# kepingbi/ProdSearch

Hardware: AMD Instinct MI355X
Metric: train (u,q,i,neg) tuples/sec at bs=384, 20 neg, d=128 (higher is better)
Workload: dtype f32 (fp32 MFMA and VALU; wide products, the fused per-replica kernels and grouped weight gradients as fp32-grade bf16x3 products: exact 3-way bf16 split of both fp32 operands, 6 of the 9 cross products as bf16 MFMAs per step, fp32 accumulation); 1 GPU; item_transformer d=128 1 layer 8 heads ff=512 uprev=20 bs=384/GPU 20 neg Q=8 W=1 P=18357 V=32387 dropout=0.10 (BASELINE configs[1]); global_batch=384, parallelism=dp1, step=sample+fwd+bwd+clip/Adam via nn.Module API (trainer.py:74-78), replicas_per_row=21

## Files before the change

### include/prodsearch_hip.h

```cpp
#ifndef PRODSEARCH_HIP_H
#define PRODSEARCH_HIP_H

#include <stddef.h>
#include <stdint.h>

#ifdef __cplusplus
extern "C" {
#endif

#define PS_MAX_LAYERS 8
#define PS_OK 0
#define PS_ERR_ARG 1
#define PS_ERR_HIP 2

typedef void* ps_stream_t;

enum { PS_MODEL_TEM = 0, PS_MODEL_QEM = 1,
       PS_MODEL_AEM = 2,
       PS_MODEL_ZAM = 3 };
enum { PS_QENC_FS = 0, PS_QENC_AVG = 1 };

typedef struct PsTemDesc {
  int32_t B;
  int32_t K;
// ... 40 lines not shown
  float *fs_w, *fs_b;
  float *pe;
  float *final_ln_g, *final_ln_b;
  PsLayerTensors layer[PS_MAX_LAYERS];
} PsTemTensors;

typedef struct PsTemBatch {
  const int64_t *query_word_idxs;
  const int64_t *target_prod_idxs;
  const int64_t *u_item_idxs;
  const int64_t *pos_iword_idxs;
  const int64_t *neg_item_idxs;
  const int64_t *neg_word_idxs;
  const int64_t *candi_prod_idxs;
} PsTemBatch;

typedef struct PsTemWsLayout {
  int64_t total_floats;
  int32_t R;
  int32_t S;
  int64_t qmean, query_emb, x;
  int64_t kp, vp, qp, attn, ctx;
  int64_t y1, ln1, a1, h1, y2, enc;
  int64_t item_scores, word_scores, loss_parts;
  int64_t denc, dx;
} PsTemWsLayout;

const char* ps_version(void);
const char* ps_last_error(void);
const char* ps_arith_info(void);
int ps_set_fuse_bwd_min(int rows);
int ps_set_item_scatter_fused(int on);
int ps_item_scatter_fused_taken(void);
int ps_set_side_mode(int mode);
int ps_side_values_in_use(void);
void ps_side_abort(void);
void ps_debug_fail_fork(int nth);
int ps_set_deterministic(int on);
int ps_gemm_x3_config(int mode, int force_shape);
int ps_gemm_f32_weight(const float* A, int lda, const float* W, int tb, float* C, int ldc, int M, int N, int K,
                       const float* bias, float alpha, ps_stream_t stream);

int ps_tem_workspace_layout(const PsTemDesc* desc, PsTemWsLayout* out);

int ps_tem_forward(const PsTemDesc* desc, const PsTemTensors* params, const PsTemBatch* batch,
                   float* workspace, float* loss3, float* loss_acc, ps_stream_t stream);
int ps_tem_forward_sampled(const PsTemDesc* desc, const PsTemTensors* params, const PsTemBatch* batch,
                           const float* alias_prob, const int32_t* alias_idx, int64_t* neg_item_out, int64_t* neg_word_out,
                           float* workspace, float* loss3, float* loss_acc, ps_stream_t stream);

int ps_tem_backward(const PsTemDesc* desc, const PsTemTensors* params, const PsTemBatch* batch,
                    float* workspace, const PsTemTensors* grads, float loss_scale,
                    const float* loss_scale_dev ,
                    ps_stream_t stream);

int ps_gather_score(const PsTemDesc* desc, const PsTemTensors* params, const PsTemBatch* batch,
                    float* workspace, ps_stream_t stream);

int ps_tem_score(const PsTemDesc* desc, const PsTemTensors* params, const PsTemBatch* batch,
                 float* workspace, float* scores, ps_stream_t stream);

int ps_sample_negatives(const PsTemDesc* desc, const float* alias_prob, const int32_t* alias_idx,
                        int64_t* neg_item_idxs, int64_t* neg_word_idxs, ps_stream_t stream);
int ps_build_alias_host(const double* dist_host, int64_t n, float* prob_host, int32_t* alias_host);

typedef struct PsAdamHyper {
// ... 199 lines not shown
```

### prodsearch_amd/_lib.py

```python
import ctypes as C
import os

from . import build as _build

PS_MAX_LAYERS = 8
PS_MODEL_TEM, PS_MODEL_QEM, PS_MODEL_AEM, PS_MODEL_ZAM = 0, 1, 2, 3
PS_QENC_FS, PS_QENC_AVG = 0, 1

_f32p = C.POINTER(C.c_float)
_i64p = C.POINTER(C.c_int64)


class PsTemDesc(C.Structure):
    _fields_ = [(n, C.c_int32) for n in ('B', 'K', 'L', 'Q', 'W', 'C', 'd', 'H', 'F', 'n_layers')] + \
               [('product_size', C.c_int64), ('vocab_size', C.c_int64)] + \
               [(n, C.c_int32) for n in ('model', 'query_encoder', 'use_pos_emb', 'use_item_pos',
                                         'bias_product', 'pos_weight', 'sep_prod_emb', 'training')] + \
               [('dropout', C.c_float), ('seed', C.c_uint64), ('step', C.c_uint64)]


LAYER_FIELDS = ('wk', 'bk', 'wv', 'bv', 'wq', 'bq', 'wo', 'bo', 'w1', 'b1', 'w2', 'b2',
                'ff_ln_g', 'ff_ln_b', 'ln_g', 'ln_b')
TOP_FIELDS = ('product_emb', 'hist_product_emb', 'word_emb', 'product_bias', 'word_bias',
              'fs_w', 'fs_b', 'pe', 'final_ln_g', 'final_ln_b')
# ... 49 lines not shown

RTM_TOP_FIELDS = ('word_emb', 'review_emb', 'seg_emb', 'fs_w', 'fs_b', 'pe', 'final_ln_g', 'final_ln_b',
                  'wo_w', 'wo_b', 'user_emb', 'product_emb', 'rev_fs_w', 'rev_fs_b')
RTM_BATCH_FIELDS = ('query_word_idxs', 'pos_prod_ridxs', 'pos_seg_idxs', 'pos_prod_rword_idxs',
                    'pos_prod_rword_masks', 'neg_prod_ridxs', 'neg_seg_idxs', 'neg_prod_rword_idxs',
                    'pos_prod_rword_idxs_pvc', 'neg_prod_rword_idxs_pvc', 'neg_word_idxs',
                    'candi_prod_ridxs', 'candi_seg_idxs', 'review_embeddings', 'pos_user_idxs', 'neg_user_idxs',
                    'pos_item_idxs', 'neg_item_idxs', 'candi_seq_user_idxs', 'candi_seq_item_idxs', 'neg_prod_rword_masks')


class PsRtmTensors(C.Structure):
    _fields_ = [(n, C.c_void_p) for n in RTM_TOP_FIELDS] + [('layer', PsLayerTensors * PS_MAX_LAYERS)]


class PsRtmBatch(C.Structure):
    _fields_ = [(n, C.c_void_p) for n in RTM_BATCH_FIELDS]


class PsRtmWsLayout(C.Structure):
    _fields_ = [('total_floats', C.c_int64)] + [(n, C.c_int32) for n in ('Bseq', 'S', 'J', 'pad_')] + \
               [(n, C.c_int64) for n in ('query_emb', 'valid', 'x', 'vec', 'cnt', 'enc', 'scores', 'weight',
                                         'pv_scores', 'dx')]


PS_RENC_PV, PS_RENC_PVC, PS_RENC_FS, PS_RENC_AVG = 0, 1, 2, 3

SYMBOLS = {
    'ps_version': (C.c_char_p, []),
    'ps_last_error': (C.c_char_p, []),
    'ps_arith_info': (C.c_char_p, []),
    'ps_set_fuse_bwd_min': (C.c_int, [C.c_int]),
    'ps_set_item_scatter_fused': (C.c_int, [C.c_int]),
    'ps_item_scatter_fused_taken': (C.c_int, []),
    'ps_set_side_mode': (C.c_int, [C.c_int]),
    'ps_side_values_in_use': (C.c_int, []),
    'ps_set_deterministic': (C.c_int, [C.c_int]),
    'ps_side_abort': (None, []),
    'ps_debug_fail_fork': (None, [C.c_int]),
    'ps_gemm_x3_config': (C.c_int, [C.c_int, C.c_int]),
    'ps_gemm_f32_weight': (C.c_int, [C.c_void_p, C.c_int, C.c_void_p, C.c_int, C.c_void_p, C.c_int, C.c_int, C.c_int, C.c_int,
                                     C.c_void_p, C.c_float, C.c_void_p]),
    'ps_tem_workspace_layout': (C.c_int, [C.POINTER(PsTemDesc), C.POINTER(PsTemWsLayout)]),
    'ps_tem_forward': (C.c_int, [C.POINTER(PsTemDesc), C.POINTER(PsTemTensors), C.POINTER(PsTemBatch),
                                 C.c_void_p, C.c_void_p, C.c_void_p, C.c_void_p]),
    'ps_tem_forward_sampled': (C.c_int, [C.POINTER(PsTemDesc), C.POINTER(PsTemTensors), C.POINTER(PsTemBatch),
                                         C.c_void_p, C.c_void_p, C.c_void_p, C.c_void_p, C.c_void_p, C.c_void_p, C.c_void_p,
                                         C.c_void_p]),
    'ps_tem_backward': (C.c_int, [C.POINTER(PsTemDesc), C.POINTER(PsTemTensors), C.POINTER(PsTemBatch),
                                  C.c_void_p, C.POINTER(PsTemTensors), C.c_float, C.c_void_p, C.c_void_p]),
    'ps_gather_score': (C.c_int, [C.POINTER(PsTemDesc), C.POINTER(PsTemTensors), C.POINTER(PsTemBatch),
                                  C.c_void_p, C.c_void_p]),
    'ps_tem_score': (C.c_int, [C.POINTER(PsTemDesc), C.POINTER(PsTemTensors), C.POINTER(PsTemBatch),
                               C.c_void_p, C.c_void_p, C.c_void_p]),
    'ps_rtm_workspace_floats': (C.c_int, [C.POINTER(PsRtmDesc), C.c_int32, C.POINTER(C.c_int64)]),
    'ps_rtm_workspace_layout': (C.c_int, [C.POINTER(PsRtmDesc), C.c_int32, C.POINTER(PsRtmWsLayout)]),
    'ps_rtm_forward': (C.c_int, [C.POINTER(PsRtmDesc), C.POINTER(PsRtmTensors), C.POINTER(PsRtmBatch),
                                 C.c_void_p, C.c_void_p, C.c_void_p]),
    'ps_rtm_backward': (C.c_int, [C.POINTER(PsRtmDesc), C.POINTER(PsRtmTensors), C.POINTER(PsRtmBatch),
                                  C.c_void_p, C.POINTER(PsRtmTensors), C.c_float, C.c_void_p, C.c_void_p]),
    'ps_rtm_score': (C.c_int, [C.POINTER(PsRtmDesc), C.POINTER(PsRtmTensors), C.POINTER(PsRtmBatch),
                               C.c_void_p, C.c_void_p, C.c_void_p]),
    'ps_rtm_review_embeddings': (C.c_int, [C.POINTER(PsRtmDesc), C.POINTER(PsRtmTensors), C.c_void_p,
                                           C.c_void_p, C.c_void_p, C.c_void_p]),
    'ps_sample_negatives': (C.c_int, [C.POINTER(PsTemDesc), C.c_void_p, C.c_void_p, C.c_void_p,
                                      C.c_void_p, C.c_void_p]),
    'ps_build_alias_host': (C.c_int, [C.c_void_p, C.c_int64, C.c_void_p, C.c_void_p]),
# ... 171 lines not shown
```

### prodsearch_amd/csrc/mlp_fused.hip

```cpp
#include "rowwise.h"
#include "x3frag.h"
#include <stdlib.h>
#ifndef TRY
#define TRY(x) do { int _rc = (x); if (_rc) return _rc; } while (0)
#endif

bool ps_fusion_enabled() {
  static const bool on = ps_env_int("PS_NO_FUSE", 0) == 0;
  return on;
}

#define MD 128
#define MBM 32
#define MT_THREADS 512
#define MLP_PF_DEFAULT 3
#define PLD 132

__device__ inline int opaque(int v) { asm volatile("" : "+v"(v)); return v; }

struct MlpTLds {
  uint16_t Xa[3][MBM * MD];
  float Ps[8][MBM * PLD];
  float vec[6][MD];
  float red[16];
// ... 356 lines not shown
template <class K>
static int set_lds_attr(K kernel, bool& done) {
  if (!done) {
    PS_CHECK_HIP(hipFuncSetAttribute(reinterpret_cast<const void*>(kernel), hipFuncAttributeMaxDynamicSharedMemorySize, (int)sizeof(MlpTLds)));
    done = true;
  }
  return PS_OK;
}

int launch_mlp_fwd_fused(const MlpFwdArgs& a, hipStream_t st) {
  PS_REQUIRE(mlp_x3_enabled(a.F) && a.M > 0, "fused mlp: F=%d M=%d (F must be 256, 512 or 1024)", a.F, a.M);
  PS_REQUIRE(a.x3.on && a.x3.fwd_wo && a.x3.fwd_ff, "fused mlp: the weight fragment streams are missing (WSplit)");
  PS_REQUIRE(!a.fold_score || mlp_fwd_can_fold_score(a.M, a.F, MD), "fused mlp: folded scoring needs <= 65535 workgroups");
  KTimeScope kt("mlp_fwd", st);
  MlpFwdArgs as = a;
  as.stamp = g_mlp_stamp;
  const dim3 grid(ps_cdiv(a.M, MBM)), block(MT_THREADS);
  static bool a1 = false, a2 = false, a4 = false;
#ifdef PS_DIAG
  static bool ad1 = false, ad2 = false, ad3 = false;
  static const int diag = ps_diag_int("PS_MLP_DIAG", 0);
  if (a.F == 512 && diag == 1) { TRY(set_lds_attr(mlp_fwd_t_kernel<2, 3, 1>, ad1)); PS_KLAUNCH((mlp_fwd_t_kernel<2, 3, 1>), grid, block, sizeof(MlpTLds), st, as); }
  else if (a.F == 512 && diag == 2) { TRY(set_lds_attr(mlp_fwd_t_kernel<2, 3, 2>, ad2)); PS_KLAUNCH((mlp_fwd_t_kernel<2, 3, 2>), grid, block, sizeof(MlpTLds), st, as); }
  else if (a.F == 512 && diag == 3) { TRY(set_lds_attr(mlp_fwd_t_kernel<2, 3, 3>, ad3)); PS_KLAUNCH((mlp_fwd_t_kernel<2, 3, 3>), grid, block, sizeof(MlpTLds), st, as); }
  else
#endif
  if (a.F == 256) { TRY(set_lds_attr(mlp_fwd_t_kernel<1, 3>, a1)); PS_KLAUNCH((mlp_fwd_t_kernel<1, 3>), grid, block, sizeof(MlpTLds), st, as); }
  else if (a.F == 512) { TRY(set_lds_attr(mlp_fwd_t_kernel<2, 3>, a2)); PS_KLAUNCH((mlp_fwd_t_kernel<2, 3>), grid, block, sizeof(MlpTLds), st, as); }
  else { TRY(set_lds_attr(mlp_fwd_t_kernel<4, 3>, a4)); PS_KLAUNCH((mlp_fwd_t_kernel<4, 3>), grid, block, sizeof(MlpTLds), st, as); }
  PS_LAUNCH_CHECK();
  return PS_OK;
}

template <int NBW, int PF, bool ISC>
__global__ __launch_bounds__(MT_THREADS, 2) void mlp_bwd_t_kernel(const MlpBwdArgs a) {
  fork_signal(a.sig, a.sigval);
  extern __shared__ float lds_raw[];
  MlpTLds& L = *reinterpret_cast<MlpTLds*>(lds_raw);
  const int tid = threadIdx.x, lane = tid & 63, wave = __builtin_amdgcn_readfirstlane(tid >> 6), l31 = lane & 31, h = lane >> 5;
  const int m0 = blockIdx.x * MBM, M = a.M, F = a.F;
  const int mrow = 4 * wave + (lane >> 4), c8 = 8 * (lane & 15);
  const int mg = m0 + mrow;
  const bool ok = mg < M;
  const uint32_t step_ctx = drop_step(a.drop_ctx), step_ff1 = drop_step(a.drop_ff1), step_ff2 = drop_step(a.drop_ff2);
  MLP_STAMP(0);
  float (*Csum)[MBM][MD] = reinterpret_cast<float (*)[MBM][MD]>(&L.Ps[2][0]);
  static_assert(3 * MBM * MD <= 3 * MBM * PLD, "column-sum scratch must fit three partial slots");

  const uint16_t* ff_stream = a.x3.bwd_ff + (size_t)(wave * NBW) * 16 * 1536;
  uint4 ring[PF][3];
#pragma unroll
  for (int s = 0; s < PF; ++s) load_frag(ring[s], ff_stream, s, lane);
  if (tid < 64) {
    const int which = tid >> 5, q = tid & 31;
    *reinterpret_cast<float4*>(&L.vec[which][4 * q]) = *reinterpret_cast<const float4*>((which == 0 ? a.gf : a.g1) + 4 * q);
  }
  float isc_e[4][2], isc_ds[4]; int isc_idx[4]; bool isc_live[4];
  if (ISC) {
#pragma unroll
    for (int r = 0; r < 4; ++r) {
      const int mr = m0 + 4 * wave + r;
      const float* er = a.enc + (size_t)(mr < M ? mr : 0) * MD + lane;
      isc_e[r][0] = er[0]; isc_e[r][1] = er[64];
    }
  }
  auto isc_add = [&](const int r) {
    float* g = a.g_product_emb + (size_t)isc_idx[r] * MD + lane;
    atomicAdd(g, isc_live[r] ? isc_ds[r] * isc_e[r][0] : 0.f);
    atomicAdd(g + 64, isc_live[r] ? isc_ds[r] * isc_e[r][1] : 0.f);
    if (a.g_product_bias && lane == 0) atomicAdd(&a.g_product_bias[isc_idx[r]], isc_ds[r]);
  };
  float x2[8], st2[2] = {0.f, 0.f};
  {
    const float* src = a.y2 + (size_t)(ok ? mg : 0) * MD + c8;
    const float4 v0 = ok ? *reinterpret_cast<const float4*>(src) : make_float4(0.f, 0.f, 0.f, 0.f);
    const float4 v1 = ok ? *reinterpret_cast<const float4*>(src + 4) : make_float4(0.f, 0.f, 0.f, 0.f);
    x2[0] = v0.x; x2[1] = v0.y; x2[2] = v0.z; x2[3] = v0.w; x2[4] = v1.x; x2[5] = v1.y; x2[6] = v1.z; x2[7] = v1.w;
    if (ok) { const float2 s2 = *reinterpret_cast<const float2*>(a.stf + 2 * (size_t)mg); st2[0] = s2.x; st2[1] = s2.y; }
  }
  float dy[8];
  if (a.item_scores) {
    const float invB = a.scale * (a.scale_dev ? *a.scale_dev : 1.f) / (float)a.B;
    const float wpos = a.pos_weight ? (float)a.K : 1.f;
    const int K1 = a.K + 1;
    const int mm = ok ? mg : 0;
    const int b = mm / K1, j = mm - b * K1;
    int64_t idx = j == 0 ? a.target[b] : a.neg_items[(size_t)b * a.K + j - 1];
    idx = idx < 0 ? a.P : (idx > a.P ? a.P : idx);
    const float sc = a.item_scores[mm];
    const float ds = ok ? (j == 0 ? wpos * (sigmoid_f(sc) - 1.f) : sigmoid_f(sc)) * invB : 0.f;
    const float* row = a.product_emb + (size_t)idx * MD + c8;
    const float4 v0 = *reinterpret_cast<const float4*>(row), v1 = *reinterpret_cast<const float4*>(row + 4);
    dy[0] = ds * v0.x; dy[1] = ds * v0.y; dy[2] = ds * v0.z; dy[3] = ds * v0.w;
    dy[4] = ds * v1.x; dy[5] = ds * v1.y; dy[6] = ds * v1.z; dy[7] = ds * v1.w;
    if (ISC) {
#pragma unroll
      for (int r = 0; r < 4; ++r) {
        isc_ds[r] = __builtin_bit_cast(float, __builtin_amdgcn_readlane(__builtin_bit_cast(int, ds), 16 * r));
        isc_idx[r] = __builtin_amdgcn_readlane((int)idx, 16 * r);
        isc_live[r] = m0 + 4 * wave + r < M && isc_idx[r] != (int)a.P;
      }
    }
  } else {
    const float* src = a.denc + (size_t)(ok ? mg : 0) * MD + c8;
    const float4 v0 = ok ? *reinterpret_cast<const float4*>(src) : make_float4(0.f, 0.f, 0.f, 0.f);
    const float4 v1 = ok ? *reinterpret_cast<const float4*>(src + 4) : make_float4(0.f, 0.f, 0.f, 0.f);
    dy[0] = v0.x; dy[1] = v0.y; dy[2] = v0.z; dy[3] = v0.w; dy[4] = v1.x; dy[5] = v1.y; dy[6] = v1.z; dy[7] = v1.w;
  }
  __syncthreads();
  MLP_STAMP(1);

  auto ln_bwd_stage = [&](const float (&dyv)[8], const float (&x)[8], const float mean, const float rstd, const int vg,
                          const bool has_res, const float (&res)[8], const DropSpec& drop, const uint32_t dstep,
                          float (&dxr)[8], float* out_dx, float* out_drop) {
    const float4 g0 = *reinterpret_cast<const float4*>(&L.vec[vg][c8]), g1 = *reinterpret_cast<const float4*>(&L.vec[vg][c8 + 4]);
    const float gg[8] = {g0.x, g0.y, g0.z, g0.w, g1.x, g1.y, g1.z, g1.w};
    float xh[8], dh[8], s1 = 0.f, s2 = 0.f;
#pragma unroll
    for (int j = 0; j < 8; ++j) {
      xh[j] = (x[j] - mean) * rstd;
      dh[j] = dyv[j] * gg[j];
      s1 += dh[j]; s2 += dh[j] * xh[j];
    }
    s1 = row16_sum(s1) * (1.f / MD);
    s2 = row16_sum(s2) * (1.f / MD);
    Philox4 rnd = {0u, 0u, 0u, 0u};
    if (drop.thr) rnd = drop_call16(drop, (uint32_t)mg, (uint32_t)(lane & 15), dstep);
    float v[8];
#pragma unroll
    for (int j = 0; j < 8; ++j) {
      float dlt = rstd * (dh[j] - s1 - xh[j] * s2);
      if (has_res) dlt += res[j];
      if (!ok) dlt = 0.f;
      dxr[j] = dlt;
// ... 39 lines not shown
#pragma unroll
    for (int j = 0; j < 8; ++j) dyz[j] = ok ? dy[j] : 0.f;
    ln_bwd_stage(dyz, x2, st2[0], st2[1], 0, false, zero, a.drop_ff2, step_ff2, dy2r, nullptr, a.do2);
  }
  __syncthreads();
  MLP_STAMP(2);
  park(a.part_f);
  __syncthreads();
  MLP_STAMP(3);

  f32x16 acc2[4];
#pragma unroll
  for (int nb = 0; nb < 4; ++nb)
#pragma unroll
    for (int r = 0; r < 16; ++r) acc2[nb][r] = 0.f;
  const int mrow_p = m0 + l31;
  const bool row_ok = mrow_p < M;
  constexpr int NS = 16 * NBW;
#pragma unroll
  for (int bi = 0; bi < NBW; ++bi) {
    const int fb = wave * NBW + bi, f0 = 32 * fb + 16 * h;
    float* tile = &L.Ps[wave][0];
    float4 a1g[4];
    tile_load(a1g, a.a1 + (size_t)m0 * F + 32 * fb, F, lane, M - m0);
    f32x16 acc1;
#pragma unroll
    for (int r = 0; r < 16; ++r) acc1[r] = 0.f;
    uint4 bq[2][3];
    read_b(bq[0], L.Xa, l31, 8 * h);
    if (ISC) {
#pragma unroll
      for (int r = 0; r < 4; ++r) if (r * NBW / 2 == 2 * bi) isc_add(r);
    }
    { if ((wave >= 4) == (bi == 0)) __builtin_amdgcn_s_setprio(2); else __builtin_amdgcn_s_setprio(1); }
#pragma unroll
    for (int t = 0; t < 8; ++t) {
      const int s = 16 * bi + t;
      if (t + 1 < 8) read_b(bq[(t + 1) & 1], L.Xa, l31, 16 * (t + 1) + 8 * h);
      __builtin_amdgcn_sched_barrier(0);
      x3_mma(acc1, ring[s % PF], bq[t & 1]);
      load_frag(ring[s % PF], ff_stream, s + PF < NS ? s + PF : NS - 1, lane);
      __builtin_amdgcn_sched_barrier(0);
    }
    { if ((wave >= 4) == (bi == 0)) __builtin_amdgcn_s_setprio(1); else __builtin_amdgcn_s_setprio(0); }
    MLP_STAMP(4 + 2 * bi);
    Philox4 r0 = {0u, 0u, 0u, 0u}, r1 = {0u, 0u, 0u, 0u};
    if (a.drop_ff1.thr) {
      r0 = drop_call16(a.drop_ff1, (uint32_t)mrow_p, (uint32_t)(f0 >> 3), step_ff1);
      r1 = drop_call16(a.drop_ff1, (uint32_t)mrow_p, (uint32_t)(f0 >> 3) + 1u, step_ff1);
    }
    float a1v[16];
    tile_load_put(tile, a1g, lane);
    tile_get(tile, a1v, l31, h);
    float dv[16];
#pragma unroll
    for (int r = 0; r < 16; ++r) {
      float g = acc1[r] * gelu_tanh_grad(a1v[r]);
      if (a.drop_ff1.thr) g *= drop_half(a.drop_ff1, r < 8 ? r0 : r1, r & 7);
      dv[r] = row_ok ? g : 0.f;
    }
    tile_put(tile + MBM * TLD, dv, l31, h);
    tile_store(tile + MBM * TLD, a.da1 + (size_t)m0 * F + 32 * fb, F, lane, M - m0);
    {
      float cs[16];
#pragma unroll
      for (int r = 0; r < 16; ++r) cs[r] = half_sum_last(dv[r]);
      if (l31 == 31) {
        float* pb = a.part_b1 + ((size_t)blockIdx.x * 3) * F + f0;
#pragma unroll
        for (int q = 0; q < 4; ++q) *reinterpret_cast<float4*>(pb + 4 * q) = make_float4(cs[4 * q], cs[4 * q + 1], cs[4 * q + 2], cs[4 * q + 3]);
      }
    }
    MLP_STAMP(5 + 2 * bi);
    { if ((wave >= 4) == (bi == 0)) __builtin_amdgcn_s_setprio(2); else __builtin_amdgcn_s_setprio(1); }
    uint4 df[2][3];
    {
      const float lo8[8] = {dv[0], dv[1], dv[2], dv[3], dv[4], dv[5], dv[6], dv[7]};
      const float hi8[8] = {dv[8], dv[9], dv[10], dv[11], dv[12], dv[13], dv[14], dv[15]};
      split8(lo8, df[0]);
      split8(hi8, df[1]);
    }
    if (ISC) {
#pragma unroll
      for (int r = 0; r < 4; ++r) if (r * NBW / 2 == 2 * bi + 1) isc_add(r);
    }
#pragma unroll
    for (int u = 0; u < 8; ++u) {
      const int s = 16 * bi + 8 + u;
      x3_mma(acc2[u & 3], ring[s % PF], df[u >> 2]);
      load_frag(ring[s % PF], ff_stream, s + PF < NS ? s + PF : NS - 1, lane);
      __builtin_amdgcn_sched_barrier(0);
    }
  }
  __builtin_amdgcn_s_setprio(0);
  MLP_STAMP(8);
  float x1[8], st1v[2] = {0.f, 0.f};
  {
    const float* src = a.y1 + (size_t)(ok ? mg : 0) * MD + c8;
    const float4 v0 = ok ? *reinterpret_cast<const float4*>(src) : make_float4(0.f, 0.f, 0.f, 0.f);
    const float4 v1 = ok ? *reinterpret_cast<const float4*>(src + 4) : make_float4(0.f, 0.f, 0.f, 0.f);
    x1[0] = v0.x; x1[1] = v0.y; x1[2] = v0.z; x1[3] = v0.w; x1[4] = v1.x; x1[5] = v1.y; x1[6] = v1.z; x1[7] = v1.w;
    if (ok) { const float2 s2 = *reinterpret_cast<const float2*>(a.st1 + 2 * (size_t)mg); st1v[0] = s2.x; st1v[1] = s2.y; }
  }
  const int kbo = wave & 3, nh = wave >> 2;
  const uint16_t* wo_stream = a.x3.bwd_wo + (size_t)(kbo * 8 + 4 * nh) * 1536;
  uint4 wof[4][3];
#pragma unroll
  for (int t = 0; t < 4; ++t) load_frag(wof[t], wo_stream, t, lane);
#pragma unroll
  for (int nb = 0; nb < 4; ++nb) dump_acc(L.Ps[wave], acc2[nb], l31, h, nb);
  __syncthreads();
  MLP_STAMP(9);

  float dl[8] = {0.f, 0.f, 0.f, 0.f, 0.f, 0.f, 0.f, 0.f};
  for (int s = 0; s < 8; ++s) {
    const float* p = &L.Ps[s][mrow * PLD + c8];
    const float4 p0 = *reinterpret_cast<const float4*>(p), p1 = *reinterpret_cast<const float4*>(p + 4);
    dl[0] += p0.x; dl[1] += p0.y; dl[2] += p0.z; dl[3] += p0.w; dl[4] += p1.x; dl[5] += p1.y; dl[6] += p1.z; dl[7] += p1.w;
  }
  __syncthreads();
  MLP_STAMP(10);
  {
    float dy1r[8];
    const bool same = a.dout == a.dy1;
// ... 1 lines not shown
  }
  __syncthreads();
  MLP_STAMP(11);
  park(a.part_1);
  {
    f32x16 acc;
#pragma unroll
    for (int r = 0; r < 16; ++r) acc[r] = 0.f;
#pragma unroll
    for (int t = 0; t < 4; ++t) {
      uint4 b[3];
      read_b(b, L.Xa, l31, 16 * (4 * nh + t) + 8 * h);
      x3_mma(acc, wof[t], b);
    }
    dump_acc(L.Ps[nh], acc, l31, h, kbo);
  }
  __syncthreads();
  MLP_STAMP(12);
  if (ok) {
    const float* p0 = &L.Ps[0][mrow * PLD + c8];
    const float* p1 = &L.Ps[1][mrow * PLD + c8];
    const float4 u0 = *reinterpret_cast<const float4*>(p0), u1 = *reinterpret_cast<const float4*>(p0 + 4);
    const float4 w0 = *reinterpret_cast<const float4*>(p1), w1 = *reinterpret_cast<const float4*>(p1 + 4);
    float* q = a.dctx + (size_t)mg * MD + c8;
    *reinterpret_cast<float4*>(q) = make_float4(u0.x + w0.x, u0.y + w0.y, u0.z + w0.z, u0.w + w0.w);
    *reinterpret_cast<float4*>(q + 4) = make_float4(u1.x + w1.x, u1.y + w1.y, u1.z + w1.z, u1.w + w1.w);
  }
  MLP_STAMP(13);
}

int mlp_bwd_fused_blocks(int M) { return ps_cdiv(M, MBM); }
int mlp_bwd_b1_rows(int M, int F) { (void)F; return ps_cdiv(M, MBM); }

int launch_mlp_bwd_fused(const MlpBwdArgs& a, hipStream_t st) {
  PS_REQUIRE(mlp_x3_enabled(a.F) && a.M > 0, "fused mlp backward: F=%d M=%d (F must be 256, 512 or 1024)", a.F, a.M);
  PS_REQUIRE(a.part_f && a.part_1 && a.part_b1, "fused mlp backward: column sums must be parked");
  PS_REQUIRE(a.x3.on && a.x3.bwd_wo && a.x3.bwd_ff, "fused mlp backward: the weight fragment streams are missing (WSplit)");
  const bool isc = a.g_product_emb != nullptr;
  PS_REQUIRE(!isc || (a.item_scores && a.enc && a.M == a.B * (a.K + 1)), "fused mlp backward: the item scatter needs the scores, enc and M = B (K + 1)");
  KTimeScope kt("mlp_bwd", st);
  MlpBwdArgs b = a;
  b.sig = nullptr; b.sigval = 0;
  b.stamp = g_mlp_stamp ? g_mlp_stamp + 128 : nullptr;
  const dim3 grid(ps_cdiv(a.M, MBM)), block(MT_THREADS);
  static bool a1 = false, a2 = false, a4 = false, s1 = false, s2 = false, s4 = false;
  if (isc) {
    if (a.F == 256) TRY(set_lds_attr(mlp_bwd_t_kernel<1, 3, true>, s1));
    else if (a.F == 512) TRY(set_lds_attr(mlp_bwd_t_kernel<2, 3, true>, s2));
    else TRY(set_lds_attr(mlp_bwd_t_kernel<4, 3, true>, s4));
  } else {
    if (a.F == 256) TRY(set_lds_attr(mlp_bwd_t_kernel<1, 3, false>, a1));
    else if (a.F == 512) TRY(set_lds_attr(mlp_bwd_t_kernel<2, 3, false>, a2));
    else TRY(set_lds_attr(mlp_bwd_t_kernel<4, 3, false>, a4));
  }
  side_take_signal(st, &b.sig, &b.sigval);
  if (isc) {
    if (a.F == 256) hipLaunchKernelGGL((mlp_bwd_t_kernel<1, 3, true>), grid, block, sizeof(MlpTLds), st, b);
    else if (a.F == 512) hipLaunchKernelGGL((mlp_bwd_t_kernel<2, 3, true>), grid, block, sizeof(MlpTLds), st, b);
    else hipLaunchKernelGGL((mlp_bwd_t_kernel<4, 3, true>), grid, block, sizeof(MlpTLds), st, b);
  } else {
    if (a.F == 256) hipLaunchKernelGGL((mlp_bwd_t_kernel<1, 3, false>), grid, block, sizeof(MlpTLds), st, b);
    else if (a.F == 512) hipLaunchKernelGGL((mlp_bwd_t_kernel<2, 3, false>), grid, block, sizeof(MlpTLds), st, b);
    else hipLaunchKernelGGL((mlp_bwd_t_kernel<4, 3, false>), grid, block, sizeof(MlpTLds), st, b);
  }
  PS_LAUNCH_CHECK();
  return PS_OK;
}
```

### prodsearch_amd/csrc/rowwise.h

```cpp
#pragma once
#include "common.h"

struct ScoreArgs {
  int B, K, W, C, R, d;
  FDiv fK1, fWK1, fC;
  int64_t P, V;
  int bias_product, pos_weight;
  const int64_t* target; const int64_t* neg_items; const int64_t* pos_words; const int64_t* neg_words;
  const int64_t* candi;
  const float* product_emb; const float* word_emb; const float* product_bias; const float* word_bias;
  const float* enc;
  float* item_scores;
  float* word_scores;
  float* loss_parts;
  float* item_terms;
  float* word_terms;
  float* loss3;
  float* loss_acc;
  float* loss_blk;
  int loss_nblk;
  float scale;
  const float* scale_dev;
  float* denc;
  int part;
// ... 220 lines not shown
};
int launch_stage(const StageArgs& a, hipStream_t st);
const void* stage_kernel_handle();
const void* loss_kernel_handle();
int score_fwd_blocks(const ScoreArgs& a);

int launch_sample(const PsTemDesc& d, const float* alias_prob, const int32_t* alias_idx, int64_t* neg_items,
                  int64_t* neg_words, hipStream_t st);

struct MlpFwdArgs {
  int M, F;
  int fan, S, qpos;
  const float* ctx; const float* xin;
  const float *wo, *bo, *g1, *be1, *w1, *b1, *w2, *b2, *gf, *bef;
  DropSpec drop_ctx, drop_ff1, drop_ff2;
  float *y1, *ln1, *st1, *a1, *h1, *y2, *stf, *enc;
  int fold_score; ScoreArgs sc;
  WSplit x3;
  unsigned long long* stamp;
};
int launch_mlp_fwd_fused(const MlpFwdArgs& a, hipStream_t st);
bool mlp_fwd_can_fold_score(int M, int F, int d);
bool mlp_x3_enabled(int F);
bool mlp_fused_serves(int d, int F);
int64_t mlp_x3_floats(int d, int F);
bool ps_fusion_enabled();

struct MlpBwdArgs {
  int M, F;
  const float* denc;
  const float* item_scores; const int64_t* target; const int64_t* neg_items; const float* product_emb;
  int B, K, pos_weight; int64_t P; float scale; const float* scale_dev;
  const float* enc; float* g_product_emb; float* g_product_bias;
  const float* y2; const float* stf; const float* gf;
  const float* y1; const float* st1; const float* g1;
  const float* a1;
  const float *wo, *w1, *w2;
  DropSpec drop_ctx, drop_ff1, drop_ff2;
  float* do2;
  float* da1;
  float* dy1;
  float* dout;
  float* dctx;
  float* part_f;
  float* part_1;
  float* part_b1;
  WSplit x3;
  uint32_t* sig; uint32_t sigval;
  unsigned long long* stamp;
};
int launch_mlp_bwd_fused(const MlpBwdArgs& a, hipStream_t st);
int mlp_bwd_fused_blocks(int M);
int mlp_bwd_b1_rows(int M, int F);
```

### prodsearch_amd/csrc/tem.hip

```cpp
#include "encoder.h"
#include "graph.h"
#include <math.h>
#include <stdarg.h>
#include <stdio.h>
#include <string.h>

static thread_local char g_err[512] = "";
void ps_set_error(const char* fmt, ...) {
  va_list ap;
  va_start(ap, fmt);
  vsnprintf(g_err, sizeof(g_err), fmt, ap);
  va_end(ap);
}
extern "C" const char* ps_last_error(void) { return g_err; }
extern "C" const char* ps_version(void) { return "prodsearch_hip 0.1 (gfx950, fp32 MFMA)"; }
bool gemm_x3_on();
extern "C" const char* ps_arith_info(void) {
  return gemm_x3_on() ? "f32 (fp32 MFMA and VALU; wide products, the fused per-replica kernels and grouped weight gradients as fp32-grade "
                        "bf16x3 products: exact 3-way bf16 split of both fp32 operands, 6 of the 9 cross products as bf16 MFMAs per step, "
                        "fp32 accumulation)"
                      : "f32 (fp32 MFMA and VALU)";
}

#include <vector>
// ... 970 lines not shown
  return PS_OK;
}

static void park_colsums(LnBwdArgs& a, float* ws, const Ws& w, ColFoldList* fold) {
  if (!fold || fold->n >= PS_MAX_COLFOLD) return;
  ColFold& f = fold->e[fold->n];
  a.partial = ws + w.lnpart + (size_t)fold->n * w.lnrows * 3 * a.d;
  f.partial = a.partial; f.nblk = ln_bwd_blocks(a.rows); f.d = a.d;
  f.dst[0] = a.dgamma; f.dst[1] = a.dbeta; f.dst[2] = a.colsum;
  ++fold->n;
}

static int& fuse_bwd_min_slot() {
  static int v = ps_env_int("PS_FUSE_BWD_MIN", 1024);
  return v;
}
extern "C" int ps_set_fuse_bwd_min(int rows) {
  const int old = fuse_bwd_min_slot();
  fuse_bwd_min_slot() = rows;
  return old;
}

static int& item_scatter_fused_slot() {
  static int v = ps_env_int("PS_ITEM_SCATTER_FUSED", 1);
  return v;
}
extern "C" int ps_set_item_scatter_fused(int on) {
  const int old = item_scatter_fused_slot();
  item_scatter_fused_slot() = on;
  return old;
}
static int g_item_scatter_taken = 0;
extern "C" int ps_item_scatter_fused_taken(void) { return g_item_scatter_taken; }

static thread_local GemmProblem g_wg3_last[4];
static thread_local int g_wg3_last_n = 0;
static thread_local bool g_wg3_defer_ok = false;
static thread_local bool g_score_words_last = false;
static int flush_wg3_last(hipStream_t st) {
  const int n = g_wg3_last_n;
  g_wg3_last_n = 0;
  return n ? run_wgrads(g_wg3_last, n, st) : PS_OK;
}
int enc_layers_backward(const PsTemDesc& D, const PsTemTensors& P, const PsTemTensors& G, const int64_t* ui,
                        const float* valid, float* ws, const Ws& w, hipStream_t st, ColFoldList* fold,
                        const ScoreArgs* score_on_side, bool rows_listed) {
  const bool drop = D.training && D.dropout > 0.f;
  const int B = D.B, d = D.d, S = w.S, NL = D.n_layers, F = D.F;
  PS_REQUIRE(G.final_ln_g && G.final_ln_b, "backward: null final LayerNorm gradient");
  LnBwdArgs f;
  memset(&f, 0, sizeof(f));
  f.dy = ws + w.denc; f.lddy = d; f.stats = ws + w.fin_stats; f.g = P.final_ln_g; f.d = d;
  f.dgamma = G.final_ln_g; f.dbeta = G.final_ln_b;
  side_set_light((int64_t)B * S * d <= ((int64_t)2 << 20));
  static const bool bwd_fuse_on = ps_env_int("PS_NO_FUSE_BWD", 0) == 0;
  const int bwd_fuse_min = fuse_bwd_min_slot();
  g_item_scatter_taken = 0;
  const bool fuse_last = NL > 0 && fold && bwd_fuse_on && ps_fusion_enabled() && w.layer[NL - 1].Sq == 1 &&
                         mlp_fused_serves(d, F) && w.wsplit && w.layer[NL - 1].M2 == w.Mf && w.Mf >= bwd_fuse_min &&
                         mlp_bwd_fused_blocks(w.Mf) <= w.lnrows && fold->n + 3 <= PS_MAX_COLFOLD;
  if (score_on_side && !(fuse_last && w.R > 1)) {
    ScoreArgs t = *score_on_side;
    t.denc = ws + w.denc;
    SideCtx* sc = side_ctx_on(st);
    if (sc && w.R > 1) {
      t.part = 1;
      TRY(launch_score_bwd(t, st));
      TRY(side_fork(st));
      t.part = 2;
      TRY(launch_score_bwd(t, sc->stream));
    } else {
      TRY(launch_score_bwd(t, st));
    }
    score_on_side = nullptr;
  }
  if (fuse_last) {
  } else if (NL > 0) {
    const LayerWs& l = w.layer[NL - 1];
    f.x = ws + l.y2; f.ldx = d; f.rows = w.Mf; f.dx = ws + w.dy2; f.lddx = d;
    f.colsum = G.layer[NL - 1].b2;
    if (drop) { f.out2 = ws + w.do2; f.drop2 = make_drop(D, PS_SITE_FF2(NL - 1)); }
    park_colsums(f, ws, w, fold);
    TRY(launch_ln_bwd(f, st));
  } else {
    PS_CHECK_HIP(hipMemsetAsync(ws + w.dx, 0, sizeof(float) * (size_t)B * S * d, st));
    f.x = ws + w.x + (size_t)w.qpos * d; f.ldx = S * d; f.rows = B;
    f.dx = ws + w.dx + (size_t)w.qpos * d; f.lddx = S * d;
    park_colsums(f, ws, w, fold);
    TRY(launch_ln_bwd(f, st));
  }
  for (int i = NL - 1; i >= 0; --i) {
    const LayerWs& l = w.layer[i];
    const PsLayerTensors& Lp = P.layer[i];
    const PsLayerTensors& Lg = G.layer[i];
    PS_REQUIRE(Lg.wk && Lg.wv && Lg.wq && Lg.wo && Lg.w1 && Lg.w2 && Lg.bk && Lg.bv && Lg.bq && Lg.bo && Lg.b1 &&
               Lg.b2 && Lg.ff_ln_g && Lg.ff_ln_b, "backward: layer %d has null gradients", i);
    const float* xin = i == 0 ? ws + w.x : ws + w.layer[i - 1].y2;
    const float* xn = ws + l.xn;
    const int ns = l.n_in * S, M2 = l.M2;
    const float* do2 = drop ? ws + w.do2 : ws + w.dy2;
    const bool fused = fuse_last && i == NL - 1;
    static const bool wgrad_early = ps_diag_int("PS_WGRAD_LATE", 0) == 0;
    if (fused) {
      MlpBwdArgs m;
      memset(&m, 0, sizeof(m));
      m.M = M2; m.F = F;
      m.denc = ws + w.denc; m.y2 = ws + l.y2; m.stf = ws + w.fin_stats; m.gf = P.final_ln_g;
      m.y1 = ws + l.y1; m.st1 = ws + l.ff_stats; m.g1 = Lp.ff_ln_g; m.a1 = ws + l.a1;
      m.wo = Lp.wo; m.w1 = Lp.w1; m.w2 = Lp.w2;
      m.drop_ctx = make_drop(D, PS_SITE_CTX(i)); m.drop_ff1 = make_drop(D, PS_SITE_FF1(i));
      m.drop_ff2 = make_drop(D, PS_SITE_FF2(i));
      if (score_on_side) {
        const ScoreArgs& sa = *score_on_side;
        m.item_scores = sa.item_scores; m.target = sa.target; m.neg_items = sa.neg_items; m.product_emb = sa.product_emb;
        m.B = sa.B; m.K = sa.K; m.pos_weight = sa.pos_weight; m.P = sa.P; m.scale = sa.scale; m.scale_dev = sa.scale_dev;
        if (item_scatter_fused_slot() != 0 && !ps_deterministic() && g_wg3_defer_ok && sa.part == 0 && sa.enc && sa.g_product_emb) {
          m.enc = sa.enc; m.g_product_emb = sa.g_product_emb;
          m.g_product_bias = sa.bias_product ? sa.g_product_bias : nullptr;
        }
      }
      m.x3 = make_wsplit(D, P, ws, w);
      m.do2 = const_cast<float*>(do2); m.da1 = ws + w.da1; m.dy1 = ws + w.dy1;
      m.dout = drop ? ws + w.do_ : ws + w.dy1; m.dctx = ws + w.dctx;
      const int nwg = mlp_bwd_fused_blocks(M2);
      {
        ColFold& c0 = fold->e[fold->n];
        m.part_f = ws + w.lnpart + (size_t)fold->n * w.lnrows * 3 * d;
        c0.partial = m.part_f; c0.nblk = nwg; c0.d = d;
        c0.dst[0] = G.final_ln_g; c0.dst[1] = G.final_ln_b; c0.dst[2] = Lg.b2;
        ++fold->n;
        ColFold& c1 = fold->e[fold->n];
        m.part_1 = ws + w.lnpart + (size_t)fold->n * w.lnrows * 3 * d;
        c1.partial = m.part_1; c1.nblk = nwg; c1.d = d;
        c1.dst[0] = Lg.ff_ln_g; c1.dst[1] = Lg.ff_ln_b; c1.dst[2] = Lg.bo;
        ++fold->n;
        ColFold& c2 = fold->e[fold->n];
        m.part_b1 = ws + w.gcpart;
        c2.partial = m.part_b1; c2.nblk = mlp_bwd_b1_rows(M2, F); c2.d = F;
        c2.dst[0] = Lg.b1; c2.dst[1] = nullptr; c2.dst[2] = nullptr;
        ++fold->n;
      }
      TRY(launch_mlp_bwd_fused(m, st));
      GemmProblem wg[1] = {gp_wgrad(do2, d, ws + l.h1, F, Lg.w2, d, F, M2)};
      GemmProblem wg1[1] = {gp_wgrad(ws + w.da1, F, ws + l.ln1, d, Lg.w1, F, d, M2)};
      GemmProblem wgo[1] = {gp_wgrad(m.dout, d, ws + l.ctx, d, Lg.wo, d, d, M2)};
      TRY(side_fork(st));
      if (score_on_side && m.g_product_emb) {
        g_score_words_last = true;
        g_item_scatter_taken = 1;
      } else if (score_on_side) {
        ScoreArgs t = *score_on_side;
        t.denc = nullptr;
        SideCtx* sc = side_ctx_on(st);
        TRY(launch_score_bwd(t, sc ? sc->stream : st));
      }
      static const int wg_group_rows = ps_diag_int("PS_WGRAD_GROUP_ROWS", (1 << 30));
      if (M2 <= wg_group_rows) {
        GemmProblem all3[3] = {wg[0], wg1[0], wgo[0]};
        TRY(side_run(all3, 3, st));
      } else {
        TRY(side_run(wg, 1, st));
        TRY(side_run(wg1, 1, st));
        TRY(side_run(wgo, 1, st));
      }
    } else {
      GemmProblem p = gp(do2, d, 0, Lp.w2, F, 1, ws + w.da1, F, M2, F, d);
      p.act = ACT_GELU_BWD; p.act_aux = ws + l.a1; p.drop = make_drop(D, PS_SITE_FF1(i)); p.colsum = Lg.b1;
      if (fold && fold->n < PS_MAX_COLFOLD && i == NL - 1) {
        ColFold& cf = fold->e[fold->n++];
        p.colsum_part = ws + w.gcpart;
        cf.partial = p.colsum_part; cf.nblk = 4 * ps_cdiv(M2, 64); cf.d = F;
        cf.dst[0] = Lg.b1; cf.dst[1] = nullptr; cf.dst[2] = nullptr;
      }
      TRY(run1(p, st));
      GemmProblem wg[1] = {gp_wgrad(do2, d, ws + l.h1, F, Lg.w2, d, F, M2)};
      GemmProblem wg1[1] = {gp_wgrad(ws + w.da1, F, ws + l.ln1, d, Lg.w1, F, d, M2)};
      GemmProblem q = gp(ws + w.da1, F, 0, Lp.w1, d, 1, ws + w.dln1, d, M2, d, F);
      TRY(run1(q, st));
      if (wgrad_early) {
        TRY(side_fork(st));
        TRY(side_run(wg, 1, st));
        TRY(side_run(wg1, 1, st));
// ... 124 lines not shown
    if (i != 0) {
      TRY(side_join(st));
      PS_REQUIRE(Lg.ln_g && Lg.ln_b, "backward: layer %d null pre-LN gradient", i);
      LnBwdArgs n;
      memset(&n, 0, sizeof(n));
      n.dy = ws + w.dxn; n.lddy = d; n.x = xin; n.ldx = d; n.stats = ws + l.pre_stats; n.g = Lp.ln_g;
      n.rows = ns; n.d = d;
      n.res.mode = RES_FANIN; n.res.ptr = ws + w.dy1; n.res.ld = d; n.res.Sq = l.Sq; n.res.fan = l.fan;
      n.res.S = S; n.res.qpos = w.qpos; res_finish(n.res);
      n.dx = ws + w.dy2; n.lddx = d;
      if (drop) { n.out2 = ws + w.do2; n.drop2 = make_drop(D, PS_SITE_FF2(i - 1)); }
      n.colsum = G.layer[i - 1].b2; n.dgamma = Lg.ln_g; n.dbeta = Lg.ln_b;
      park_colsums(n, ws, w, fold);
      TRY(launch_ln_bwd(n, st));
    }
  }
  return PS_OK;
}

static int tem_backward_impl(const PsTemDesc* desc, const PsTemTensors* params, const PsTemBatch* batch,
                             float* ws, const PsTemTensors* grads, float loss_scale, const float* loss_scale_dev,
                             ps_stream_t stream);
extern "C" int ps_tem_backward(const PsTemDesc* desc, const PsTemTensors* params, const PsTemBatch* batch,
                               float* ws, const PsTemTensors* grads, float loss_scale, const float* loss_scale_dev,
                               ps_stream_t stream) {
  const int rc = tem_backward_impl(desc, params, batch, ws, grads, loss_scale, loss_scale_dev, stream);
  if (rc != PS_OK) { side_abort(); enc_clear_call_flags(); }
  return rc;
}
static int tem_backward_impl(const PsTemDesc* desc, const PsTemTensors* params, const PsTemBatch* batch,
                             float* ws, const PsTemTensors* grads, float loss_scale, const float* loss_scale_dev,
                             ps_stream_t stream) {
  enc_clear_call_flags();
  g_item_scatter_taken = 0;
  PS_REQUIRE(desc && params && batch && ws && grads, "backward: null argument");
  PsTemDesc D = *desc;
  D.C = 0;
  Ws w;
  TRY(make_ws(D, w));
  hipStream_t st = (hipStream_t)stream;
  const PsTemTensors& P = *params;
  const PsTemTensors& G = *grads;
  const bool tem = D.model == PS_MODEL_TEM;
  const bool drop = D.training && D.dropout > 0.f;
  const int B = D.B, d = D.d, S = w.S, NL = tem ? D.n_layers : 0, F = D.F;
  const float* hist = D.sep_prod_emb ? P.hist_product_emb : P.product_emb;
  float* ghist = D.sep_prod_emb ? G.hist_product_emb : G.product_emb;
  const bool word_grad = G.word_emb != nullptr;
  PS_REQUIRE(G.product_emb && G.word_bias && ghist && hist, "backward: null table gradient");
  PS_REQUIRE(!D.bias_product || G.product_bias, "backward: null product_bias gradient");

  ScoreArgs s;
  fill_score(D, P, *batch, ws, w, s);
  s.scale = loss_scale; s.scale_dev = loss_scale_dev; s.denc = ws + w.denc;
  s.g_product_emb = G.product_emb; s.g_word_emb = G.word_emb; s.g_product_bias = G.product_bias;
  s.g_word_bias = G.word_bias;
  static const bool score_side_on = ps_diag_int("PS_SCORE_BWD_MAIN", 0) == 0;
  const bool score_deferred = tem && NL > 0 && w.R > 1 && score_side_on;
  if (!score_deferred) TRY(launch_score_bwd(s, st));

  const float* wp_w[PS_WPLANES_MAX]; int wp_r[PS_WPLANES_MAX], wp_c[PS_WPLANES_MAX];
  const int wp_n = wplane_list(D, P, w, wp_w, wp_r, wp_c);
  WPlaneScope wplanes(st, wp_w, wp_r, wp_c, wp_n);
  ColFoldList fold;
  fold.n = 0;
  bool score_words_last = false;
  const float* dqe = ws + w.denc;
// ... 265 lines not shown
```

Measured before the change: 36.90 million tuples/s.

## Fuse word-score gradient scatter into the fused MLP backward kernel

Moves the word-score backward work (word embedding, word bias and target product-embedding gradient atomics) into the fused MLP backward kernel, which already carries the item scatter. Word and product rows are prefetched and the atomics are interleaved between MFMA steps. This removes the separate word-score backward launch and its re-read of scores and indices. The cost is extra registers and atomics inside a latency-sensitive MFMA loop, plus more template variants.

```diff
diff --git a/include/prodsearch_hip.h b/include/prodsearch_hip.h
--- a/include/prodsearch_hip.h
+++ b/include/prodsearch_hip.h
@@ -96,6 +96,8 @@
 int ps_set_fuse_bwd_min(int rows);
 int ps_set_item_scatter_fused(int on);
 int ps_item_scatter_fused_taken(void);
+int ps_set_word_scatter_fused(int on);
+int ps_word_scatter_fused_taken(void);
 int ps_set_side_mode(int mode);
 int ps_side_values_in_use(void);
 void ps_side_abort(void);
diff --git a/prodsearch_amd/_lib.py b/prodsearch_amd/_lib.py
--- a/prodsearch_amd/_lib.py
+++ b/prodsearch_amd/_lib.py
@@ -105,6 +105,8 @@
     'ps_set_fuse_bwd_min': (C.c_int, [C.c_int]),
     'ps_set_item_scatter_fused': (C.c_int, [C.c_int]),
     'ps_item_scatter_fused_taken': (C.c_int, []),
+    'ps_set_word_scatter_fused': (C.c_int, [C.c_int]),
+    'ps_word_scatter_fused_taken': (C.c_int, []),
     'ps_set_side_mode': (C.c_int, [C.c_int]),
     'ps_side_values_in_use': (C.c_int, []),
     'ps_set_deterministic': (C.c_int, [C.c_int]),
diff --git a/prodsearch_amd/csrc/mlp_fused.hip b/prodsearch_amd/csrc/mlp_fused.hip
--- a/prodsearch_amd/csrc/mlp_fused.hip
+++ b/prodsearch_amd/csrc/mlp_fused.hip
@@ -412,7 +412,10 @@
   return PS_OK;
 }
 
-template <int NBW, int PF, bool ISC>
+#ifndef PS_WSC_PLACE
+#define PS_WSC_PLACE 1
+#endif
+template <int NBW, int PF, bool ISC, int WSC = 0>
 __global__ __launch_bounds__(MT_THREADS, 2) void mlp_bwd_t_kernel(const MlpBwdArgs a) {
   fork_signal(a.sig, a.sigval);
   extern __shared__ float lds_raw[];
@@ -449,6 +452,52 @@
     atomicAdd(g, isc_live[r] ? isc_ds[r] * isc_e[r][0] : 0.f);
     atomicAdd(g + 64, isc_live[r] ? isc_ds[r] * isc_e[r][1] : 0.f);
     if (a.g_product_bias && lane == 0) atomicAdd(&a.g_product_bias[isc_idx[r]], isc_ds[r]);
+  };
+  static_assert(!WSC || ISC, "the word tasks ride with the item scatter");
+  constexpr int WGR = NBW == 1 ? 2 : 1;
+  constexpr int WPL = NBW == 4 ? 0 : PS_WSC_PLACE;
+  float wsc_ds[4], wsc_w[WGR][2] = {}, wsc_p[WGR][2] = {}, wsc_s[2][2] = {};
+  int wsc_idx[4], wsc_tb[4], wsc_tb1 = 0; bool wsc_second[4];
+  auto wsc_request = [&](const int g) __attribute__((always_inline)) {
+#pragma unroll
+    for (int q = 0; q < WGR; ++q) {
+      const int r = WGR * g + q;
+      const float* wr = a.word_emb + (size_t)wsc_idx[r] * MD + lane;
+      wsc_w[q][0] = wr[0]; wsc_w[q][1] = wr[64];
+      if (WSC == 1) {
+        const float* pr = a.product_emb + (size_t)wsc_tb[r] * MD + lane;
+        wsc_p[q][0] = pr[0]; wsc_p[q][1] = pr[64];
+      }
+    }
+  };
+  auto wsc_add = [&](const int g) __attribute__((always_inline)) {
+    float w[WGR][2], p[WGR][2];
+#pragma unroll
+    for (int q = 0; q < WGR; ++q) { w[q][0] = wsc_w[q][0]; w[q][1] = wsc_w[q][1]; p[q][0] = wsc_p[q][0]; p[q][1] = wsc_p[q][1]; }
+    if (WGR * (g + 1) < 4) wsc_request(g + 1);
+#pragma unroll
+    for (int q = 0; q < WGR; ++q) {
+      const int r = WGR * g + q;
+      const bool second = wsc_second[r];
+      const float t0 = wsc_ds[r] * w[q][0], t1 = wsc_ds[r] * w[q][1];
+      wsc_s[0][0] += second ? 0.f : t0; wsc_s[0][1] += second ? 0.f : t1;
+      wsc_s[1][0] += second ? t0 : 0.f; wsc_s[1][1] += second ? t1 : 0.f;
+      if (WSC == 1) {
+        const bool live = wsc_idx[r] != (int)(a.V - 1);
+        float* gw = a.g_word_emb + (size_t)wsc_idx[r] * MD + lane;
+        atomicAdd(gw, live ? wsc_ds[r] * p[q][0] : 0.f);
+        atomicAdd(gw + 64, live ? wsc_ds[r] * p[q][1] : 0.f);
+      }
+      if (lane == 0) atomicAdd(&a.g_word_bias[wsc_idx[r]], wsc_ds[r]);
+    }
+  };
+  auto wsc_target_add = [&]() __attribute__((always_inline)) {
+    const int tb0 = wsc_tb[0], tb1 = wsc_tb1;
+    float* g0 = a.g_product_emb + (size_t)tb0 * MD + lane;
+    float* g1 = a.g_product_emb + (size_t)tb1 * MD + lane;
+    const bool l0 = tb0 != (int)a.P, l1 = tb1 != (int)a.P;
+    atomicAdd(g0, l0 ? wsc_s[0][0] : 0.f); atomicAdd(g0 + 64, l0 ? wsc_s[0][1] : 0.f);
+    atomicAdd(g1, l1 ? wsc_s[1][0] : 0.f); atomicAdd(g1 + 64, l1 ? wsc_s[1][1] : 0.f);
   };
   float x2[8], st2[2] = {0.f, 0.f};
   {
@@ -480,6 +529,35 @@
         isc_idx[r] = __builtin_amdgcn_readlane((int)idx, 16 * r);
         isc_live[r] = m0 + 4 * wave + r < M && isc_idx[r] != (int)a.P;
       }
+    }
+    if (WSC) {
+      const int64_t vp = a.V - 1;
+      const int64_t pw = a.pos_words[b];
+      const int nwi = b * a.K + j - 1;
+      const int64_t nw = a.neg_words[nwi < 0 ? 0 : nwi];
+      int64_t wi = j == 0 ? pw : nw;
+      wi = wi < 0 ? vp : (wi > vp ? vp : wi);
+      int64_t tb = a.target[b];
+      tb = tb < 0 ? a.P : (tb > a.P ? a.P : tb);
+      const float sw = a.word_scores[mm];
+      const float dsw = ok && pw != vp ? (j == 0 ? sigmoid_f(sw) - 1.f : sigmoid_f(sw)) * invB : 0.f;
+#pragma unroll
+      for (int r = 0; r < 4; ++r) {
+        wsc_ds[r] = __builtin_bit_cast(float, __builtin_amdgcn_readlane(__builtin_bit_cast(int, dsw), 16 * r));
+        wsc_idx[r] = __builtin_amdgcn_readlane((int)wi, 16 * r);
+        wsc_tb[r] = __builtin_amdgcn_readlane((int)tb, 16 * r);
+      }
+      {
+        const int b0 = __builtin_amdgcn_readlane(b, 0), b1 = __builtin_amdgcn_readlane(b, 16), b2 = __builtin_amdgcn_readlane(b, 32),
+                  b3 = __builtin_amdgcn_readlane(b, 48);
+        const int t1 = wsc_tb[1], t2 = wsc_tb[2], t3 = wsc_tb[3];
+        wsc_second[0] = false; wsc_second[1] = b1 != b0; wsc_second[2] = b2 != b0; wsc_second[3] = b3 != b0;
+        int tsel = t3;
+        if (b2 != b0) tsel = t2;
+        if (b1 != b0) tsel = t1;
+        wsc_tb1 = tsel;
+      }
+      wsc_request(0);
     }
   } else {
     const float* src = a.denc + (size_t)(ok ? mg : 0) * MD + c8;
@@ -585,6 +663,10 @@
 #pragma unroll
       for (int r = 0; r < 4; ++r) if (r * NBW / 2 == 2 * bi) isc_add(r);
     }
+    if (WSC && WPL == 0) {
+#pragma unroll
+      for (int g = 0; g < 4 / WGR; ++g) if (g * WGR * NBW / 2 == 2 * bi) wsc_add(g);
+    }
     { if ((wave >= 4) == (bi == 0)) __builtin_amdgcn_s_setprio(2); else __builtin_amdgcn_s_setprio(1); }
 #pragma unroll
     for (int t = 0; t < 8; ++t) {
@@ -594,6 +676,10 @@
       x3_mma(acc1, ring[s % PF], bq[t & 1]);
       load_frag(ring[s % PF], ff_stream, s + PF < NS ? s + PF : NS - 1, lane);
       __builtin_amdgcn_sched_barrier(0);
+      if (WSC && WPL == 1 && t == 3) {
+#pragma unroll
+        for (int g = 0; g < 4 / WGR; ++g) if (g * WGR * NBW / 2 == 2 * bi) wsc_add(g);
+      }
     }
     { if ((wave >= 4) == (bi == 0)) __builtin_amdgcn_s_setprio(1); else __builtin_amdgcn_s_setprio(0); }
     MLP_STAMP(4 + 2 * bi);
@@ -637,12 +723,21 @@
 #pragma unroll
       for (int r = 0; r < 4; ++r) if (r * NBW / 2 == 2 * bi + 1) isc_add(r);
     }
+    if (WSC && WPL == 0) {
+#pragma unroll
+      for (int g = 0; g < 4 / WGR; ++g) if (g * WGR * NBW / 2 == 2 * bi + 1) wsc_add(g);
+    }
 #pragma unroll
     for (int u = 0; u < 8; ++u) {
       const int s = 16 * bi + 8 + u;
       x3_mma(acc2[u & 3], ring[s % PF], df[u >> 2]);
       load_frag(ring[s % PF], ff_stream, s + PF < NS ? s + PF : NS - 1, lane);
       __builtin_amdgcn_sched_barrier(0);
+      if (WSC && WPL == 1 && u == 3) {
+#pragma unroll
+        for (int g = 0; g < 4 / WGR; ++g) if (g * WGR * NBW / 2 == 2 * bi + 1) wsc_add(g);
+      }
+      if (WSC && bi == NBW - 1 && u == 5) wsc_target_add();
     }
   }
   __builtin_amdgcn_s_setprio(0);
@@ -710,37 +805,37 @@
 int mlp_bwd_fused_blocks(int M) { return ps_cdiv(M, MBM); }
 int mlp_bwd_b1_rows(int M, int F) { (void)F; return ps_cdiv(M, MBM); }
 
+typedef void (*MlpBwdKernel)(const MlpBwdArgs);
+template <int NBW>
+static MlpBwdKernel mlp_bwd_pick(int form) {
+  switch (form) {
+    case 1: return mlp_bwd_t_kernel<NBW, 3, true, 0>;
+    case 2: return mlp_bwd_t_kernel<NBW, 3, true, 1>;
+    case 3: return mlp_bwd_t_kernel<NBW, 3, true, 2>;
+    default: return mlp_bwd_t_kernel<NBW, 3, false, 0>;
+  }
+}
+
 int launch_mlp_bwd_fused(const MlpBwdArgs& a, hipStream_t st) {
   PS_REQUIRE(mlp_x3_enabled(a.F) && a.M > 0, "fused mlp backward: F=%d M=%d (F must be 256, 512 or 1024)", a.F, a.M);
   PS_REQUIRE(a.part_f && a.part_1 && a.part_b1, "fused mlp backward: column sums must be parked");
   PS_REQUIRE(a.x3.on && a.x3.bwd_wo && a.x3.bwd_ff, "fused mlp backward: the weight fragment streams are missing (WSplit)");
   const bool isc = a.g_product_emb != nullptr;
   PS_REQUIRE(!isc || (a.item_scores && a.enc && a.M == a.B * (a.K + 1)), "fused mlp backward: the item scatter needs the scores, enc and M = B (K + 1)");
+  const int wsc = a.g_word_bias ? (a.g_word_emb ? 1 : 2) : 0;
+  PS_REQUIRE(!wsc || (isc && a.pos_words && a.neg_words && a.word_scores && a.word_emb && a.V > 0),
+             "fused mlp backward: the word tasks need the item scatter, the word index arrays, scores and table");
   KTimeScope kt("mlp_bwd", st);
   MlpBwdArgs b = a;
   b.sig = nullptr; b.sigval = 0;
   b.stamp = g_mlp_stamp ? g_mlp_stamp + 128 : nullptr;
   const dim3 grid(ps_cdiv(a.M, MBM)), block(MT_THREADS);
-  static bool a1 = false, a2 = false, a4 = false, s1 = false, s2 = false, s4 = false;
-  if (isc) {
-    if (a.F == 256) TRY(set_lds_attr(mlp_bwd_t_kernel<1, 3, true>, s1));
-    else if (a.F == 512) TRY(set_lds_attr(mlp_bwd_t_kernel<2, 3, true>, s2));
-    else TRY(set_lds_attr(mlp_bwd_t_kernel<4, 3, true>, s4));
-  } else {
-    if (a.F == 256) TRY(set_lds_attr(mlp_bwd_t_kernel<1, 3, false>, a1));
-    else if (a.F == 512) TRY(set_lds_attr(mlp_bwd_t_kernel<2, 3, false>, a2));
-    else TRY(set_lds_attr(mlp_bwd_t_kernel<4, 3, false>, a4));
-  }
+  const int form = isc ? 1 + wsc : 0, nbi = a.F == 256 ? 0 : (a.F == 512 ? 1 : 2);
+  const MlpBwdKernel kernel = nbi == 0 ? mlp_bwd_pick<1>(form) : (nbi == 1 ? mlp_bwd_pick<2>(form) : mlp_bwd_pick<4>(form));
+  static bool attr_done[3][4] = {};
+  TRY(set_lds_attr(kernel, attr_done[nbi][form]));
   side_take_signal(st, &b.sig, &b.sigval);
-  if (isc) {
-    if (a.F == 256) hipLaunchKernelGGL((mlp_bwd_t_kernel<1, 3, true>), grid, block, sizeof(MlpTLds), st, b);
-    else if (a.F == 512) hipLaunchKernelGGL((mlp_bwd_t_kernel<2, 3, true>), grid, block, sizeof(MlpTLds), st, b);
-    else hipLaunchKernelGGL((mlp_bwd_t_kernel<4, 3, true>), grid, block, sizeof(MlpTLds), st, b);
-  } else {
-    if (a.F == 256) hipLaunchKernelGGL((mlp_bwd_t_kernel<1, 3, false>), grid, block, sizeof(MlpTLds), st, b);
-    else if (a.F == 512) hipLaunchKernelGGL((mlp_bwd_t_kernel<2, 3, false>), grid, block, sizeof(MlpTLds), st, b);
-    else hipLaunchKernelGGL((mlp_bwd_t_kernel<4, 3, false>), grid, block, sizeof(MlpTLds), st, b);
-  }
+  hipLaunchKernelGGL(kernel, grid, block, sizeof(MlpTLds), st, b);
   PS_LAUNCH_CHECK();
   return PS_OK;
 }
diff --git a/prodsearch_amd/csrc/rowwise.h b/prodsearch_amd/csrc/rowwise.h
--- a/prodsearch_amd/csrc/rowwise.h
+++ b/prodsearch_amd/csrc/rowwise.h
@@ -276,6 +276,8 @@
   const float* item_scores; const int64_t* target; const int64_t* neg_items; const float* product_emb;
   int B, K, pos_weight; int64_t P; float scale; const float* scale_dev;
   const float* enc; float* g_product_emb; float* g_product_bias;
+  const int64_t* pos_words; const int64_t* neg_words; const float* word_scores; const float* word_emb;
+  float* g_word_emb; float* g_word_bias; int64_t V;
   const float* y2; const float* stf; const float* gf;
   const float* y1; const float* st1; const float* g1;
   const float* a1;
diff --git a/prodsearch_amd/csrc/tem.hip b/prodsearch_amd/csrc/tem.hip
--- a/prodsearch_amd/csrc/tem.hip
+++ b/prodsearch_amd/csrc/tem.hip
@@ -1026,6 +1026,17 @@
 }
 static int g_item_scatter_taken = 0;
 extern "C" int ps_item_scatter_fused_taken(void) { return g_item_scatter_taken; }
+static int& word_scatter_fused_slot() {
+  static int v = ps_env_int("PS_WORD_SCATTER_FUSED", 1);
+  return v;
+}
+extern "C" int ps_set_word_scatter_fused(int on) {
+  const int old = word_scatter_fused_slot();
+  word_scatter_fused_slot() = on;
+  return old;
+}
+static int g_word_scatter_taken = 0;
+extern "C" int ps_word_scatter_fused_taken(void) { return g_word_scatter_taken; }
 
 static thread_local GemmProblem g_wg3_last[4];
 static thread_local int g_wg3_last_n = 0;
@@ -1049,7 +1060,7 @@
   side_set_light((int64_t)B * S * d <= ((int64_t)2 << 20));
   static const bool bwd_fuse_on = ps_env_int("PS_NO_FUSE_BWD", 0) == 0;
   const int bwd_fuse_min = fuse_bwd_min_slot();
-  g_item_scatter_taken = 0;
+  g_item_scatter_taken = 0; g_word_scatter_taken = 0;
   const bool fuse_last = NL > 0 && fold && bwd_fuse_on && ps_fusion_enabled() && w.layer[NL - 1].Sq == 1 &&
                          mlp_fused_serves(d, F) && w.wsplit && w.layer[NL - 1].M2 == w.Mf && w.Mf >= bwd_fuse_min &&
                          mlp_bwd_fused_blocks(w.Mf) <= w.lnrows && fold->n + 3 <= PS_MAX_COLFOLD;
@@ -1111,6 +1122,10 @@
         if (item_scatter_fused_slot() != 0 && !ps_deterministic() && g_wg3_defer_ok && sa.part == 0 && sa.enc && sa.g_product_emb) {
           m.enc = sa.enc; m.g_product_emb = sa.g_product_emb;
           m.g_product_bias = sa.bias_product ? sa.g_product_bias : nullptr;
+          if (word_scatter_fused_slot() != 0 && sa.W == 1 && sa.K >= 2 && sa.g_word_bias && sa.word_scores) {
+            m.pos_words = sa.pos_words; m.neg_words = sa.neg_words; m.word_scores = sa.word_scores; m.word_emb = sa.word_emb;
+            m.g_word_emb = sa.g_word_emb; m.g_word_bias = sa.g_word_bias; m.V = sa.V;
+          }
         }
       }
       m.x3 = make_wsplit(D, P, ws, w);
@@ -1140,8 +1155,9 @@
       GemmProblem wgo[1] = {gp_wgrad(m.dout, d, ws + l.ctx, d, Lg.wo, d, d, M2)};
       TRY(side_fork(st));
       if (score_on_side && m.g_product_emb) {
-        g_score_words_last = true;
+        g_score_words_last = m.g_word_bias == nullptr;
         g_item_scatter_taken = 1;
+        g_word_scatter_taken = m.g_word_bias ? 1 : 0;
       } else if (score_on_side) {
         ScoreArgs t = *score_on_side;
         t.denc = nullptr;
@@ -1332,7 +1348,7 @@
                              float* ws, const PsTemTensors* grads, float loss_scale, const float* loss_scale_dev,
                              ps_stream_t stream) {
   enc_clear_call_flags();
-  g_item_scatter_taken = 0;
+  g_item_scatter_taken = 0; g_word_scatter_taken = 0;
   PS_REQUIRE(desc && params && batch && ws && grads, "backward: null argument");
   PsTemDesc D = *desc;
   D.C = 0;
```

Result: slower. 32.84 million tuples/s (-11.0%).
